# vsxen/inspektor-gadget

Measured on AMD Instinct MI355X. Metric: events aggregated/sec (filter+group-by+top-K) at 1/2/4/8 MI355X; % HBM peak, higher is better.
Workload: dtype u64; 1 GPU; top-tcp: filter family in {AF_INET, AF_INET6}, group-by ip_key_t(saddr,daddr,mntns,pid,comm,lport,dport,family) sum sent/recv, stable top-20 by [-sent,-recv]; events_per_gpu=100000000, keys_per_gpu=1000000, topk=20, groups_per_gpu=991489, batches=21, claims_per_interval=0, parallelism=single GPU

## Files before the change

include/igx.h:

```cpp
#ifndef IGX_H
#define IGX_H

#include <stddef.h>
#include <stdint.h>

#ifdef __cplusplus
extern "C" {
#endif

#define IGX_OK 0
#define IGX_ENOENT (-2)
#define IGX_EIO (-5)
#define IGX_ENOMEM (-12)
#define IGX_EINVAL (-22)
#define IGX_ENOSPC (-28)
#define IGX_ENOTSUP (-95)

enum igx_kind {
    IGX_KIND_INT = 0,
    IGX_KIND_UINT = 1,
    IGX_KIND_FLOAT = 2,
    IGX_KIND_BYTES = 3,
    IGX_KIND_BOOL = 4,
    IGX_KIND_OTHER = 5
// ... 142 lines not shown
int igx_groupby_finalize(igx_table *t, igx_table_view *view);
typedef struct {
    uint32_t form;
    uint32_t region;
    uint32_t part_left;
    uint32_t exact_left;
    uint32_t sm_probers;
    uint32_t loaders;
    uint64_t rows;
    uint32_t miss_permille;
    uint32_t persist;
    uint64_t claims;
    uint64_t gen_keys;
} igx_groupby_info_t;
int igx_groupby_info(igx_table *t, igx_groupby_info_t *out);
int igx_groupby_rowplan(igx_table *t);
int igx_groupby_rowplan_match(const uint32_t *key_widths, uint32_t nkeys, const igx_agg *aggs,
                              uint32_t naggs, const igx_col *cols, uint32_t ncols,
                              const uint32_t *key_cols, const igx_pred *preds, uint32_t npreds,
                              const uint8_t *valid, uint32_t idx_col);
int igx_groupby_finalize_async(igx_table *t, igx_table_view *view);
int igx_groupby_wait(igx_table *t, uint64_t *n_groups);
int igx_groupby_gather(igx_table *t, const uint32_t *idx, uint64_t k, uint8_t *out_rows);
int igx_groupby_select_ge(igx_table *t, uint32_t agg, uint64_t threshold, uint32_t *out_slots,
                          uint64_t cap, uint64_t *d_count);
int igx_groupby_lookup(igx_table *t, const uint8_t *keys, uint32_t key_stride, uint64_t n,
                       uint8_t *out_rows, uint8_t *found);
int igx_groupby_reset(igx_table *t);
enum igx_gb_mode { IGX_GB_AUTO = 0, IGX_GB_CACHED = 1, IGX_GB_DIRECT = 2, IGX_GB_PART = 3 };
int igx_groupby_set_mode(igx_table *t, uint32_t mode);
// ... 188 lines not shown
```

inspektor-gadget_amd/_abi.py:

```python
import ctypes as C
import os

HERE = os.path.dirname(os.path.abspath(__file__))
LIB_PATH = os.environ.get("IGX_LIB") or os.path.join(HERE, "libigx.so")
if os.environ.get("IGX_LIB"):
    import sys as _sys
    print(f"inspektor-gadget_amd: IGX_LIB={LIB_PATH}", file=_sys.stderr, flush=True)

IGX_OK = 0
IGX_ENOENT = -2
IGX_EIO = -5
IGX_ENOMEM = -12
IGX_EINVAL = -22
IGX_ENOSPC = -28
IGX_ENOTSUP = -95

KIND_INT, KIND_UINT, KIND_FLOAT, KIND_BYTES, KIND_BOOL, KIND_OTHER = range(6)
CMP_EQ, CMP_REGEX, CMP_LT, CMP_LE, CMP_GT, CMP_GE, CMP_IN = range(7)
COL_VIRTUAL, COL_EXTRACTOR = 1, 2
NO_COL = 0xFFFFFFFF
MAX_REF = 256
AGG_COUNT, AGG_SUM = 0, 1
FILTER_ANY, FILTER_NIL_MATCH = 1, 2
GB_AUTO, GB_CACHED, GB_DIRECT, GB_PART = 0, 1, 2, 3
# ... 19 lines not shown
    _fields_ = [("col", C.c_uint32), ("cmp", C.c_uint32), ("negate", C.c_uint32),
                ("ref_len", C.c_uint32), ("ref", C.c_uint8 * MAX_REF),
                ("guard_col", C.c_uint32), ("guard_len", C.c_uint32), ("guard_ref", C.c_uint8 * 8)]


class SortKey(C.Structure):
    _fields_ = [("ptr", C.c_void_p), ("width", C.c_uint32), ("kind", C.c_uint32),
                ("desc", C.c_uint32), ("col", C.c_uint32)]


class GroupbyInfo(C.Structure):
    _fields_ = [("form", C.c_uint32), ("region", C.c_uint32), ("part_left", C.c_uint32),
                ("exact_left", C.c_uint32), ("sm_probers", C.c_uint32), ("loaders", C.c_uint32),
                ("rows", C.c_uint64), ("miss_permille", C.c_uint32), ("persist", C.c_uint32),
                ("claims", C.c_uint64), ("gen_keys", C.c_uint64)]


class Agg(C.Structure):
    _fields_ = [("kind", C.c_uint32), ("col", C.c_uint32), ("cond_col", C.c_uint32),
                ("out_width", C.c_uint32), ("cond_val", C.c_uint64), ("divisor", C.c_uint64)]


class TableView(C.Structure):
    _fields_ = [("n_groups", C.c_uint64), ("n_slots", C.c_uint64), ("key_bytes", C.c_uint32),
                ("key_stride", C.c_uint32), ("val_stride", C.c_uint32), ("naggs", C.c_uint32),
                ("keys", C.c_void_p),
                ("aggs", C.c_void_p * 16), ("first_idx", C.c_void_p), ("groups", C.c_void_p),
                ("d_n_groups", C.c_void_p)]


# ... 60 lines not shown
                              C.POINTER(SortKey), C.POINTER(_U32), C.POINTER(_U32)]),
    ("igx_sort_perm", _I, [_VP, C.POINTER(SortKey), _U32, _U64, _VP, _VP, _VP]),
    ("igx_sort_perm_ex", _I, [_VP, C.POINTER(SortKey), _U32, _U64, _VP, _VP, _VP, _VP]),
    ("igx_sort_perm_dn", _I, [_VP, C.POINTER(SortKey), _U32, _U64, _VP, _VP, _VP, _VP, _VP]),
    ("igx_topk", _I, [_VP, C.POINTER(SortKey), _U32, _U64, _VP, _U32, _VP]),
    ("igx_groupby_create", _I, [_VP, C.POINTER(_U32), _U32, C.POINTER(Agg), _U32, _U64,
                                C.POINTER(_VP)]),
    ("igx_groupby_update", _I, [_VP, C.POINTER(Col), _U32, C.POINTER(_U32), C.POINTER(Pred),
                                _U32, _U64, _U64]),
    ("igx_groupby_update_ex", _I, [_VP, C.POINTER(Col), _U32, C.POINTER(_U32), C.POINTER(Pred),
                                   _U32, _VP, _U32, _U64, _U64]),
    ("igx_groupby_finalize", _I, [_VP, C.POINTER(TableView)]),
    ("igx_groupby_finalize_async", _I, [_VP, C.POINTER(TableView)]),
    ("igx_groupby_wait", _I, [_VP, C.POINTER(C.c_uint64)]),
    ("igx_groupby_info", _I, [_VP, C.POINTER(GroupbyInfo)]),
    ("igx_groupby_rowplan", _I, [_VP]),
    ("igx_groupby_rowplan_match", _I, [C.POINTER(_U32), _U32, C.POINTER(Agg), _U32, C.POINTER(Col), _U32,
                                       C.POINTER(_U32), C.POINTER(Pred), _U32, _VP, _U32]),
    ("igx_groupby_gather", _I, [_VP, _VP, _U64, _VP]),
    ("igx_groupby_select_ge", _I, [_VP, _U32, _U64, _VP, _U64, _VP]),
    ("igx_groupby_lookup", _I, [_VP, _VP, _U32, _U64, _VP, _VP]),
    ("igx_groupby_sort", _I, [_VP, C.POINTER(TSortKey), _U32, _U32, _VP]),
    ("igx_segment_fsum", _I, [_VP, _VP, _U32, _U32, _VP, _U64, _VP, _VP, _U32, _VP]),
    ("igx_ip_text", _I, [_VP, _VP, _U32, _VP, _U32, _VP, _U64, _VP]),
    ("igx_groupby_reset", _I, [_VP]),
    ("igx_groupby_set_mode", _I, [_VP, _U32]),
    ("igx_groupby_destroy", _I, [_VP]),
    ("igx_groupby_debug_counts", _I, [_VP, _VP]),
    ("igx_groupby_topk_counts", _I, [_VP, _VP]),
    ("igx_np_mark", _I, [_VP, _VP, _VP, _VP, _VP, _U64, _VP]),
# ... 76 lines not shown
```

inspektor-gadget_amd/csrc/k_gb_cached.hip:

```cpp
#include "k_gb_table.h"

namespace {

constexpr uint32_t ST_EMPTY = 0xFFFFFFFFu;
constexpr uint32_t ST_BUSY = 0xFFFFFFFEu;
constexpr uint32_t GHOST = 1024;

template <int KW>
struct LdsCache {
    static constexpr int KP = (KW + 3) & ~3;
    uint32_t *tag;
    uint32_t *st;
    uint32_t *key;
    uint64_t *agg;
    uint64_t *first;
    uint32_t *ghost;
    uint32_t E;
    uint32_t nsets;
};

template <int KW>
__device__ __forceinline__ bool lds_key_eq(const LdsCache<KW> &c, uint32_t e, const uint32_t (&k)[KW]) {
    constexpr int NQ = LdsCache<KW>::KP / 4;
    const uint4 *p = reinterpret_cast<const uint4 *>(c.key) + (uint64_t)e * (LdsCache<KW>::KP / 4);
// ... 180 lines not shown
        ++lines;
    }
    const uint64_t nlive = (uint64_t)__popcll(__ballot(live));
    if (lane == 0) {
        atomicAdd(a.dbg_cnt + base, (unsigned long long)nlive);
        atomicAdd(a.dbg_cnt + base + 1, (unsigned long long)nmin);
        atomicAdd(a.dbg_cnt + base + 2, (unsigned long long)recs);
        atomicAdd(a.dbg_cnt + base + 3, (unsigned long long)lines);
    }
}

template <bool DBG>
__device__ __forceinline__ void ring_serve(const GbArgs &a, const Ring &r, uint32_t lane) {
    uint32_t head = 0;
    [[maybe_unused]] uint32_t prev_last = 0xFFFFFFFFu;
    for (;;) {
        const uint32_t t = __hip_atomic_load(&r.ctl[0], __ATOMIC_ACQUIRE, __HIP_MEMORY_SCOPE_WORKGROUP);
        if (t == head) {
            if (__hip_atomic_load(&r.ctl[2], __ATOMIC_ACQUIRE, __HIP_MEMORY_SCOPE_WORKGROUP) == NWAVES - 1 - a.nl &&
                __hip_atomic_load(&r.ctl[0], __ATOMIC_ACQUIRE, __HIP_MEMORY_SCOPE_WORKGROUP) == head)
                break;
            __builtin_amdgcn_s_sleep(2);
            if (DBG && (a.dbg & 65536u) && lane == 0) atomicAdd(a.dbg_cnt + 7, 1ull);
            continue;
        }
        const uint32_t n = min(t - head, 64u);
        uint32_t slot = 0xFFFFFFFFu, what = 0;
        if (lane < n) {
            const uint32_t p = head + lane;
            uint64_t w;
            uint32_t spins = 0;
            while (((uint32_t)((w = __hip_atomic_load(reinterpret_cast<uint64_t *>(&r.lo[p % ARING]),
                                                      __ATOMIC_ACQUIRE, __HIP_MEMORY_SCOPE_WORKGROUP)) >> 32) &
                    ~15u) != ring_lap(p)) {
                __builtin_amdgcn_s_sleep(1);
                if (++spins > SPIN_LIMIT) { atomicOr(a.err, 16u); break; }
            }
            const uint64_t val = r.hi[p % ARING];
            slot = (uint32_t)w;
            what = (uint32_t)(w >> 32) & 15u;
            if (DBG && (a.dbg & 131072u)) {
                if (what == WHAT_MIN) *rec_first(a, slot) = val;
                else *rec_agg(a, slot, (int)what) = val;
            } else if (!(DBG && (a.dbg & 4u))) {
                if (what == WHAT_MIN) gmin(rec_first(a, slot), val);
                else gadd(rec_agg(a, slot, (int)what), val);
            }
        }
        if (DBG && (a.dbg & 262144u)) {
            const bool live = lane < n;
            atomics_account(a, live, slot, what == WHAT_MIN, lane, 8);
            for (uint32_t g = 0; g < 3; ++g) {
                const uint32_t sh = 5 - g;
                uint64_t todo = __ballot(live);
                uint64_t cnt = 0;
                while (todo) {
                    const uint32_t l = (uint32_t)__ffsll((long long)todo) - 1;
                    const uint32_t s0 = __shfl(slot, (int)l), k0 = __shfl(what == WHAT_MIN ? 1u : 0u, (int)l);
                    todo &= ~__ballot(live && slot == s0 && (what == WHAT_MIN ? 1u : 0u) == k0 && (lane >> sh) == (l >> sh));
                    ++cnt;
                }
                if (lane == 0) atomicAdd(a.dbg_cnt + 13 + g, (unsigned long long)cnt);
            }
            const uint32_t first_slot = __shfl(slot, 0), last_slot = __shfl(slot, (int)(n - 1));
            if (lane == 0 && first_slot == prev_last) atomicAdd(a.dbg_cnt + 12, 1ull);
            prev_last = last_slot;
        }
        head += n;
        if (lane == 0) __hip_atomic_store(&r.ctl[1], head, __ATOMIC_RELEASE, __HIP_MEMORY_SCOPE_WORKGROUP);
    }
}

constexpr uint32_t MRING = 256;

template <int KW, int NA>
struct MissRing {
    static constexpr int KQ = LdsCache<KW>::KP / 4;
    static constexpr int EQ = KQ + 1 + (NA + 1) / 2;
    uint4 *cell;
    uint32_t *seq;
    uint32_t *ctl;
    uint32_t *err;
    unsigned long long *waits;
};
// ... 794 lines not shown
    (void)igx_groupby_reset(st);
    GbArgs b = a;
    b.n = S;
    b.naggs = 1;
    b.vcount[0] = 1;
    b.hascond[0] = 0;
    b.valid = a.valid;
    bind_records(st, b);
    b.dbg = 0;
    b.sm = 0;
    b.direct = 0;
    b.nl = NL_DEFAULT;
    b.seeds = nullptr;
    b.seed_gep = nullptr;
    b.nseeds = 0;
    st->rows_fed = S;
    st->fin_since_update = false;
    st->interval_direct = st->interval_part = false;
    st->occb_dirty = true;
    launch_gb_as<L, false, 2, true>(ctx, b, (uint32_t)std::max<uint64_t>(1, std::min<uint64_t>((S + GTB - 1) / GTB,
                                                                                           (uint64_t)ctx->num_cus)));
    IGX_HIP(ctx, hipGetLastError());
    int rc = igx_groupby_finalize_async(st, nullptr);
    if (rc) return rc;
    igx_tsortkey key{};
    key.src = IGX_TSRC_AGG;
    key.index = 0;
    key.desc = 1;
    rc = igx_groupby_sort(st, &key, 1, E, t->seed_slots);
    if (rc) return rc;
// ... 40 lines not shown
```

inspektor-gadget_amd/csrc/k_gb_table.h:

```cpp
#pragma once

#include <algorithm>
#include <cstdlib>
#include <cstring>
#include <type_traits>
#include <string>
#include <utility>
#include <vector>

#include <thread>

#include "k_common.h"

#ifndef IGX_GB_STREAM_NT
#define IGX_GB_STREAM_NT 1
#endif
#if IGX_GB_STREAM_NT
#define IGX_STREAM_LOAD(p) __builtin_nontemporal_load(p)
#else
#define IGX_STREAM_LOAD(p) (*(p))
#endif
template <bool NT, class T>
__device__ __forceinline__ T stream_ld(const T *p) {
    if constexpr (NT) return IGX_STREAM_LOAD(p);
// ... 65 lines not shown
    uint32_t vrec_words;
    uint32_t vrec_total;
    uint32_t *err;
    uint32_t *occ;
    uint8_t *occb;
    uint64_t ep;
    uint64_t *gen;
    uint64_t rmask;
    uint32_t sshift;
    uint32_t max_probe;
    uint32_t dbg;
    unsigned long long *dbg_cnt;
    const uint32_t *seeds;
    const uint64_t *seed_gep;
    uint32_t nseeds;
};

__device__ __forceinline__ uint32_t nh_const(int i) {
    return 0x9E3779B9u * (uint32_t)(2 * i + 1) + 0x7F4A7C15u;
}

template <int KW>
__device__ __forceinline__ uint64_t hash_key(const uint32_t (&k)[KW]) {
    uint64_t h = 0x243F6A8885A308D3ull ^ (uint64_t)KW;
#pragma unroll
    for (int w = 0; w < KW; w += 2) {
        const uint32_t a = k[w] + nh_const(w);
        const uint32_t b = ((w + 1 < KW) ? k[w + 1] : 0u) + nh_const(w + 1);
        h += (uint64_t)a * (uint64_t)b;
    }
    h ^= h >> 33;
// ... 606 lines not shown
    uint32_t miss_pm = 0;
    bool rowplan_on = true;
    int rowplan_last = 0;
    uint32_t mode = IGX_GB_AUTO;
    uint32_t direct_left = 0;
    uint32_t region_off = 0;
    bool interval_region = false;
    bool interval_direct = false;
    bool interval_part = false;
    uint32_t *p_recs = nullptr;
    size_t p_recs_bytes = 0;
    uint32_t *p_cnt = nullptr;
    size_t p_cnt_bytes = 0;
    uint8_t *p_mask = nullptr;
    size_t p_mask_bytes = 0;
    uint64_t host_groups = 0;
    uint64_t *fin_host = nullptr;
    uint64_t *fin_dev = nullptr;
    uint64_t fin_seq = 0;
    bool fin_pending = false;
    int fin_status = 0;
    uint64_t fin_status_seq = 0;
    struct {
        uint64_t rows_fed;
        bool direct, part, region, probe;
        uint64_t sampled;
    } fin_snap{};
    bool interval_probe = false;
    uint64_t probe_rows = 0;
    unsigned long long *dbg_cnt = nullptr;
// ... 77 lines not shown

inline int grow(igx_ctx *ctx, void **p, size_t *have, size_t need) {
    if (*have >= need) return IGX_OK;
    IGX_HIP(ctx, hipStreamSynchronize(ctx->stream));
    (void)hipFree(*p);
    *p = nullptr;
    *have = 0;
    IGX_HIP(ctx, hipMalloc(p, need));
    *have = need;
    return IGX_OK;
}

int gb_launch_cached(igx_table *t, GbArgs &a, uint32_t blocks);
int gb_launch_estimate(igx_table *t, const GbArgs &a, uint32_t blocks, uint64_t nsample);
int gb_seeds_compute(igx_table *t, const GbArgs &a);
int gb_launch_direct(igx_table *t, GbArgs &a);
int gb_launch_part(igx_table *t, GbArgs &a);
void gb_cached_load();
void gb_direct_load();
void gb_part_load();
int fin_collect(igx_table *t, uint64_t *n_groups);
```

inspektor-gadget_amd/csrc/k_groupby.hip:

```cpp
#include "k_gb_table.h"

namespace {

__global__ void k_table_clear(uint8_t *krec, uint32_t krec_len, uint32_t koff, uint64_t ns) {
    const uint64_t stride = (uint64_t)gridDim.x * blockDim.x;
    for (uint64_t i = (uint64_t)blockIdx.x * blockDim.x + threadIdx.x; i < ns; i += stride)
        *reinterpret_cast<uint4 *>(krec + i * krec_len + koff) = make_uint4(0, 0, 0, 0);
}

constexpr int CT = 256 * 32;

__global__ __launch_bounds__(256) void k_occ_from_tags(const uint8_t *__restrict__ krec, uint32_t krec_len,
                                                       uint32_t koff, uint64_t ns, uint64_t ep,
                                                       uint32_t *__restrict__ occ) {
    const uint64_t w = (uint64_t)blockIdx.x * 256 + threadIdx.x;
    if (w * 32 >= ns) return;
    uint32_t m = 0;
#pragma unroll 8
    for (uint32_t b = 0; b < 32; ++b) {
        const uint64_t s = w * 32 + b;
        const uint64_t t = s < ns ? *reinterpret_cast<const uint64_t *>(krec + s * krec_len + koff) : 0;
        m |= ((t & EP_MAX) == ep ? 1u : 0u) << b;
    }
    occ[w] |= m;
// ... 30 lines not shown

__device__ __forceinline__ void fin_export(const uint32_t *err, uint64_t total, uint64_t *host, uint64_t seq, uint64_t ep) {
    const uint64_t e0 = *reinterpret_cast<const volatile uint64_t *>(err);
    const uint64_t e1 = *reinterpret_cast<const volatile uint64_t *>(err + 2);
    volatile uint64_t *gen = reinterpret_cast<volatile uint64_t *>(const_cast<uint32_t *>(err)) + GEN_WORD;
    const bool fresh = gen[0] == ep;
    const uint64_t claims = fresh ? total : gen[2];
    const uint64_t keys = (uint32_t)e0 ? ~0ull : (fresh ? total : gen[1] + claims);
    gen[1] = keys;
    gen[2] = 0;
    __hip_atomic_store(host, e0, __ATOMIC_RELAXED, __HIP_MEMORY_SCOPE_SYSTEM);
    __hip_atomic_store(host + 1, e1, __ATOMIC_RELAXED, __HIP_MEMORY_SCOPE_SYSTEM);
    __hip_atomic_store(host + 2, total, __ATOMIC_RELAXED, __HIP_MEMORY_SCOPE_SYSTEM);
    __hip_atomic_store(host + 4, claims, __ATOMIC_RELAXED, __HIP_MEMORY_SCOPE_SYSTEM);
    __hip_atomic_store(host + 5, keys, __ATOMIC_RELAXED, __HIP_MEMORY_SCOPE_SYSTEM);
    __threadfence_system();
    __hip_atomic_store(host + 3, seq, __ATOMIC_RELEASE, __HIP_MEMORY_SCOPE_SYSTEM);
}

__global__ __launch_bounds__(1024) void k_slots_scan(uint32_t *__restrict__ v, uint64_t m, uint64_t *__restrict__ total,
                                                     const uint32_t *__restrict__ err, uint64_t *__restrict__ host,
                                                     uint64_t seq, uint64_t ep) {
    __shared__ uint32_t part[1024];
    const uint64_t per = (m + 1023) / 1024;
    const uint64_t b = threadIdx.x * per, e = min(m, b + per);
    uint32_t s = 0;
    for (uint64_t i = b; i < e; ++i) s += v[i];
    part[threadIdx.x] = s;
    __syncthreads();
    for (int d = 1; d < 1024; d <<= 1) {
// ... 67 lines not shown
    const uint32_t *groups;
    const uint64_t *ng;
    uint64_t *vrec;
    uint32_t vw, may;
};
__global__ __launch_bounds__(256) void k_reset_clear(uint32_t *__restrict__ occ, uint64_t nwords,
                                                     uint32_t *__restrict__ err, uint4 *__restrict__ occb,
                                                     uint64_t nb16, ResetGen rg) {
    const uint64_t i = (uint64_t)blockIdx.x * 256 + threadIdx.x;
    const uint64_t stride = (uint64_t)gridDim.x * 256;
    const uint64_t n4 = nwords / 4;
    for (uint64_t q = i; q < n4; q += stride) reinterpret_cast<uint4 *>(occ)[q] = make_uint4(0, 0, 0, 0);
    for (uint64_t q = i; q < nb16; q += stride) occb[q] = make_uint4(0, 0, 0, 0);
    if (i < (nwords & 3)) occ[n4 * 4 + i] = 0;
    if (i < 4) err[i] = 0;
    const bool cont = rg.may && rg.gen[1] <= rg.limit;
    if (cont) {
        constexpr int RU = 8;
        const uint64_t ng = *rg.ng;
        const uint32_t qs = rg.vw == 1 ? 0u : (uint32_t)__builtin_ctz(rg.vw / 2);
        const uint64_t total = ng << qs;
        const uint32_t *__restrict__ groups = rg.groups;
        uint64_t *__restrict__ vrec = rg.vrec;
        for (uint64_t j0 = i; j0 < total; j0 += RU * stride) {
            uint32_t slot[RU];
#pragma unroll
            for (int u = 0; u < RU; ++u) {
                const uint64_t j = j0 + u * stride;
                slot[u] = j < total ? groups[j >> qs] : 0u;
            }
// ... 175 lines not shown
    t->cap = capacity;
    uint64_t slotf = 8;
    if (const char *d = std::getenv("IGX_GB_SLOTF")) slotf = std::max<uint64_t>(5, std::strtoul(d, nullptr, 0));
    uint64_t ns = 1024;
    while (ns * 4 < slotf * capacity) ns <<= 1;
    t->nslots = ns;
    t->sbits = (uint32_t)__builtin_ctzll(ns);
    t->rbits = std::max<uint32_t>(10, t->sbits > 14 ? t->sbits - 14 : 0);
    t->wide = ns * t->krec_len >= (1ull << 32);
    if (const char *d = std::getenv("IGX_GB_WIDE"))
        t->wide = t->wide || std::strtoul(d, nullptr, 0) != 0;
    const uint64_t tiles = (ns + CT - 1) / CT;
    hipError_t e = hipMalloc(&t->krec, ns * t->krec_len);
    if (e == hipSuccess) e = hipMemsetAsync(t->krec, 0, ns * t->krec_len, ctx->stream);
    if (e == hipSuccess) e = hipMalloc(&t->vrec, ns * t->vrec_len);
    if (e == hipSuccess) e = hipMalloc(&t->err, 64);
    if (e == hipSuccess) e = hipMemsetAsync(t->err, 0, 64, ctx->stream);
    if (e == hipSuccess) e = hipMalloc(&t->groups, ns * 4);
    if (e == hipSuccess) e = hipMalloc(&t->tile_cnt, tiles * 4);
    t->occ_words = (ns + 31) / 32;
    if (e == hipSuccess) e = hipMalloc(&t->occ, t->occ_words * 4);
    if (e == hipSuccess) e = hipMalloc(&t->occb, t->occ_words * 32);
    if (e == hipSuccess) e = hipMemsetAsync(t->occb, 0, t->occ_words * 32, ctx->stream);
    if (e == hipSuccess) t->n_groups = reinterpret_cast<uint64_t *>(t->err + 4);
    if (e == hipSuccess) e = hipMalloc(&t->dbg_cnt, 256);
    if (e == hipSuccess)
        e = hipHostMalloc(reinterpret_cast<void **>(&t->fin_host), 64, hipHostMallocMapped | hipHostMallocCoherent);
    if (e == hipSuccess) e = hipHostGetDevicePointer(reinterpret_cast<void **>(&t->fin_dev), t->fin_host, 0);
    if (e == hipSuccess) std::fill(t->fin_host, t->fin_host + 8, 0ull);
    if (e == hipSuccess) e = hipMemsetAsync(t->dbg_cnt, 0, 256, ctx->stream);
    if (e != hipSuccess) {
        igx_groupby_destroy(t);
        return igx_fail(ctx, IGX_ENOMEM, "groupby_create: %s", hipGetErrorString(e));
    }
    if (const char *m = std::getenv("IGX_GB_MODE")) {
        const unsigned long v = std::strtoul(m, nullptr, 0);
        if (v <= IGX_GB_PART && !(t->wide && v == IGX_GB_CACHED)) t->mode = (uint32_t)v;
    }
    if (const char *m = std::getenv("IGX_GB_PERSIST")) t->persist = std::strtoul(m, nullptr, 0) != 0;
    if (const char *m = std::getenv("IGX_GB_SEED")) t->seed_on = std::strtoul(m, nullptr, 0) != 0;
    *out = t;
    return igx_groupby_reset(t);
}

// ... 48 lines not shown
    (void)hipFree(t->krec);
    (void)hipFree(t->vrec);
    (void)hipFree(t->err);
    (void)hipFree(t->groups);
    (void)hipFree(t->tile_cnt);
    (void)hipFree(t->occ);
    (void)hipFree(t->occb);
    (void)hipFree(t->dbg_cnt);
    (void)hipFree(t->seeds);
    (void)hipFree(t->seed_slots);
    (void)hipFree(t->seed_gep);
    if (t->seed_tab) igx_groupby_destroy(t->seed_tab);
    (void)hipFree(t->p_recs);
    (void)hipFree(t->p_cnt);
    (void)hipFree(t->p_mask);
    for (auto &h : t->tk) (void)hipFree(h.slots);
    (void)hipFree(t->tk_state);
    for (auto *p : t->text) (void)hipFree(p);
    if (t->fin_host) (void)hipHostFree(t->fin_host);
    delete t;
    return IGX_OK;
}

constexpr uint64_t DIRECT_MISS_PCT = 90;
constexpr uint64_t MORE_PROBERS_ON_PM = 390;
constexpr uint64_t MORE_PROBERS_OFF_PM = 370;
constexpr uint32_t DIRECT_RUN = 16;
constexpr uint64_t PROBE_ROWS = 16u << 20;
constexpr uint32_t SEED_EVERY = 16;
constexpr uint64_t SEED_MIN_ROWS = 8u << 20;
// ... 37 lines not shown
                uint32_t every = SEED_EVERY;
                if (const char *e = std::getenv("IGX_GB_SEED_EVERY"))
                    every = std::max<uint32_t>(1, (uint32_t)std::strtoul(e, nullptr, 0));
                if (gb_seeds_compute(t, a) == IGX_OK) t->seed_left = every;
                else t->nseeds = 0;
            }
            --t->seed_left;
            t->interval_seeded = t->nseeds > 0;
        }
    }
    if (t->interval_seeded) {
        a.seeds = t->seeds;
        a.seed_gep = t->seed_gep;
        a.nseeds = t->nseeds;
    }
    return gb_launch_cached(t, a, blocks);
}

extern "C" int igx_groupby_set_mode(igx_table *t, uint32_t mode) {
    if (!t) return IGX_EINVAL;
    if (mode > IGX_GB_PART) return igx_fail(t->ctx, IGX_EINVAL, "groupby_set_mode: mode %u", mode);
    if (t->wide && mode == IGX_GB_CACHED)
        return igx_fail(t->ctx, IGX_ENOTSUP, "groupby_set_mode: the cached form is not available on a wide table "
                                             "(%llu slots x %u B of key records; 64-bit record addressing)",
                        (unsigned long long)t->nslots, t->krec_len);
    t->mode = mode;
    t->direct_left = 0;
    return IGX_OK;
}

extern "C" int igx_groupby_update(igx_table *t, const igx_col *cols, uint32_t ncols, const uint32_t *key_cols,
// ... 363 lines not shown
    for (uint32_t x = 0; x < 16; ++x) view->aggs[x] = x < t->naggs ? t->vrec + 1 + x : nullptr;
    view->first_idx = t->vrec;
    view->groups = t->groups;
    view->d_n_groups = t->n_groups;
}

static int fin_apply(igx_table *t) {
    igx_ctx *ctx = t->ctx;
    const uint64_t *h = t->fin_host;
    const uint32_t err = reinterpret_cast<const uint32_t *>(h)[0];
    const uint64_t misses = h[1];
    const uint64_t ng = h[2];
    const uint32_t spilled = reinterpret_cast<const uint32_t *>(h)[1];
    t->claims_last = h[4];
    t->gen_keys = h[5];
    if (h[4] == ng || h[5] == ~0ull) t->seed_left = 0;
    const auto &f = t->fin_snap;
    if (spilled && f.region) t->region_off = DIRECT_RUN + 1;
    t->host_groups = ng;
    if (f.rows_fed >= 1000000 && !f.direct && !f.part) {
        t->prefer_sm = misses * 10 > f.rows_fed * 7;
        t->miss_pm = (uint32_t)(misses * 1000 / f.rows_fed);
        t->more_probers = t->miss_pm > (t->more_probers ? MORE_PROBERS_OFF_PM : MORE_PROBERS_ON_PM);
        if (t->mode == IGX_GB_AUTO && misses * 100 > f.rows_fed * DIRECT_MISS_PCT) t->direct_left = DIRECT_RUN;
    }
    if (f.probe && f.sampled && t->mode == IGX_GB_AUTO && misses * 100 > f.sampled * DIRECT_MISS_PCT)
        t->direct_left = DIRECT_RUN;
    if (err) return igx_fail(ctx, IGX_ENOSPC, "groupby: table full or probe failure (err=%u)", err);
    if (ng > t->cap)
        return igx_fail(ctx, IGX_ENOSPC, "groupby: %llu distinct keys exceed capacity %llu",
// ... 67 lines not shown
extern "C" int igx_groupby_info(igx_table *t, igx_groupby_info_t *out) {
    if (!t || !out) return IGX_EINVAL;
    std::memset(out, 0, sizeof *out);
    if (t->rows_fed)
        out->form = t->interval_part ? IGX_GB_PART : (t->interval_direct ? IGX_GB_DIRECT : IGX_GB_CACHED);
    out->region = t->interval_part && t->interval_region ? 1u : 0u;
    out->part_left = t->direct_left;
    out->exact_left = t->region_off;
    out->sm_probers = t->prefer_sm ? 1u : 0u;
    out->loaders = t->more_probers ? NL_DEFAULT - 1 : NL_DEFAULT;
    out->miss_permille = t->miss_pm;
    out->rows = t->rows_fed;
    out->claims = t->claims_last;
    out->gen_keys = t->gen_keys;
    out->persist = t->persist ? 1u : 0u;
    return IGX_OK;
}

static uint64_t agg_out_mask(const igx_table *t, uint32_t x) {
    const uint32_t ow = t->aggs[x].out_width;
    return (ow == 0 || ow >= 8) ? ~0ull : ((1ull << (8 * ow)) - 1);
}
static AggMasks agg_masks(const igx_table *t) {
    AggMasks am{};
    for (uint32_t x = 0; x < t->naggs; ++x) {
        const uint64_t m = agg_out_mask(t, x);
        am.m[2 * x] = (uint32_t)m;
        am.m[2 * x + 1] = (uint32_t)(m >> 32);
    }
    return am;
// ... 197 lines not shown
```

inspektor-gadget_amd/engine.py:

```python
import ctypes as C
import os
import math

from . import _abi
from ._abi import Agg, Col, Pred, SortKey, TableView, IgxError
from .runtime import context, ptr, col_of, dtype_kind, torch_mod

TCP_FIELDS = (("saddr", "u8x16"), ("daddr", "u8x16"), ("mntns", "u64"), ("pid", "u32"),
              ("comm", "u8x16"), ("lport", "u16"), ("dport", "u16"), ("family", "u16"),
              ("size", "u32"), ("dir", "u8"))
OPEN_FIELDS = (("pid", "u32"), ("uid", "u32"), ("mntns", "u64"), ("comm", "u8x16"),
               ("ret", "i64"), ("fd", "i64"), ("err", "i64"), ("path", "u32"))
BIO_FIELDS = (("dev", "u32"), ("cont", "u32"), ("delta", "i64"))
NP_FIELDS = (("src", "u32"), ("peer", "u32"), ("port", "u16"), ("pkt", "u8"), ("type", "u8"),
             ("proto", "u8"), ("hostip", "u32"), ("raddr", "u32"))
FILE_FIELDS = (("inode", "u64"), ("dev", "u32"), ("pid", "u32"), ("tid", "u32"), ("op", "u8"),
               ("count", "u32"))


def zipf_cdf(G: int, s: float):
    import numpy as np
    k = np.arange(1, G + 1, dtype=np.float64)
    c = np.cumsum(k ** (-s))
    c /= c[-1]
# ... 171 lines not shown
                                              ptr(valid), _abi.NO_COL if idx_col is None else idx_col,
                                              n, base_idx))

    def wait(self):
        n = C.c_uint64()
        self.ctx.check(self.ctx.L.igx_groupby_wait(self.h, C.byref(n)))
        if getattr(self, "fin", None) is not None:
            self.fin["n_groups"] = n.value
        return n.value

    def info(self):
        from ._abi import GroupbyInfo
        v = GroupbyInfo()
        self.ctx.check(self.ctx.L.igx_groupby_info(self.h, C.byref(v)))
        return {f: getattr(v, f) for f, _ in GroupbyInfo._fields_ if f != "pad"}

    def rowplan(self):
        return int(self.ctx.L.igx_groupby_rowplan(self.h))

    def reset(self):
        self.ctx.check(self.ctx.L.igx_groupby_reset(self.h))

    def set_mode(self, mode):
        self.ctx.check(self.ctx.L.igx_groupby_set_mode(self.h, mode))

    def finalize(self, sync=True):
        v = TableView()
        if sync:
            self.ctx.check(self.ctx.L.igx_groupby_finalize(self.h, C.byref(v)))
        else:
# ... 576 lines not shown
```

Before: 34.49 billion events/s.

## Log ring-server aggregate adds and reduce them via bucketed partition pass

Rather than issuing a scattered global atomic add per aggregate update in the cached ring server, the server writes compact (slot, agg, value) records to a per-workgroup log. Two follow-up kernels partition the log by slot bucket in shared memory and then reduce each bucket with LDS atomics before one global add per touched accumulator. Records that are too large or that overflow the log or a bucket fall back to direct atomics, and the fallback counts are reported through a new stats API. This aims to replace random HBM atomic traffic with streaming writes and reads, at the cost of extra buffers, two extra kernel launches and more total bytes moved.

```diff
diff --git a/include/igx.h b/include/igx.h
--- a/include/igx.h
+++ b/include/igx.h
@@ -180,6 +180,13 @@
     uint64_t gen_keys;
 } igx_groupby_info_t;
 int igx_groupby_info(igx_table *t, igx_groupby_info_t *out);
+typedef struct {
+    uint64_t logged;
+    uint64_t fallback_value;
+    uint64_t fallback_log_full;
+    uint64_t fallback_bucket_full;
+} igx_groupby_log_stats_t;
+int igx_groupby_log_stats(igx_table *t, igx_groupby_log_stats_t *out);
 int igx_groupby_rowplan(igx_table *t);
 int igx_groupby_rowplan_match(const uint32_t *key_widths, uint32_t nkeys, const igx_agg *aggs,
                               uint32_t naggs, const igx_col *cols, uint32_t ncols,
diff --git a/inspektor-gadget_amd/_abi.py b/inspektor-gadget_amd/_abi.py
--- a/inspektor-gadget_amd/_abi.py
+++ b/inspektor-gadget_amd/_abi.py
@@ -57,6 +57,11 @@
                 ("exact_left", C.c_uint32), ("sm_probers", C.c_uint32), ("loaders", C.c_uint32),
                 ("rows", C.c_uint64), ("miss_permille", C.c_uint32), ("persist", C.c_uint32),
                 ("claims", C.c_uint64), ("gen_keys", C.c_uint64)]
+
+
+class GroupbyLogStats(C.Structure):
+    _fields_ = [("logged", C.c_uint64), ("fallback_value", C.c_uint64),
+                ("fallback_log_full", C.c_uint64), ("fallback_bucket_full", C.c_uint64)]
 
 
 class Agg(C.Structure):
@@ -147,6 +152,7 @@
     ("igx_groupby_finalize_async", _I, [_VP, C.POINTER(TableView)]),
     ("igx_groupby_wait", _I, [_VP, C.POINTER(C.c_uint64)]),
     ("igx_groupby_info", _I, [_VP, C.POINTER(GroupbyInfo)]),
+    ("igx_groupby_log_stats", _I, [_VP, C.POINTER(GroupbyLogStats)]),
     ("igx_groupby_rowplan", _I, [_VP]),
     ("igx_groupby_rowplan_match", _I, [C.POINTER(_U32), _U32, C.POINTER(Agg), _U32, C.POINTER(Col), _U32,
                                        C.POINTER(_U32), C.POINTER(Pred), _U32, _VP, _U32]),
diff --git a/inspektor-gadget_amd/csrc/k_gb_cached.hip b/inspektor-gadget_amd/csrc/k_gb_cached.hip
--- a/inspektor-gadget_amd/csrc/k_gb_cached.hip
+++ b/inspektor-gadget_amd/csrc/k_gb_cached.hip
@@ -218,6 +218,9 @@
 __device__ __forceinline__ void ring_serve(const GbArgs &a, const Ring &r, uint32_t lane) {
     uint32_t head = 0;
     [[maybe_unused]] uint32_t prev_last = 0xFFFFFFFFu;
+    const bool logging = !DBG && a.log != nullptr;
+    uint64_t *lg = a.log + (uint64_t)blockIdx.x * a.log_cap;
+    uint32_t lpos = 0, n_logged = 0, n_value = 0, n_full = 0;
     for (;;) {
         const uint32_t t = __hip_atomic_load(&r.ctl[0], __ATOMIC_ACQUIRE, __HIP_MEMORY_SCOPE_WORKGROUP);
         if (t == head) {
@@ -229,6 +232,7 @@
             continue;
         }
         const uint32_t n = min(t - head, 64u);
+        const bool room = logging && lpos + n <= a.log_cap;
         uint32_t slot = 0xFFFFFFFFu, what = 0;
         if (lane < n) {
             const uint32_t p = head + lane;
@@ -243,12 +247,28 @@
             const uint64_t val = r.hi[p % ARING];
             slot = (uint32_t)w;
             what = (uint32_t)(w >> 32) & 15u;
-            if (DBG && (a.dbg & 131072u)) {
+            bool logged = false;
+            if (logging && what != WHAT_MIN) {
+                const bool small = (val >> 32) == 0;
+                const bool fits = small && slot < LOG_SLOT_LIMIT;
+                if (!small) ++n_value;
+                if (fits && !room) ++n_full;
+                logged = fits && room;
+                n_logged += logged ? 1u : 0u;
+            }
+            if (room)
+                __builtin_nontemporal_store(logged ? log_record(slot, what, (uint32_t)val) : ~0ull, lg + lpos + lane);
+            if (logged) {
+            } else if (DBG && (a.dbg & 131072u)) {
                 if (what == WHAT_MIN) *rec_first(a, slot) = val;
                 else *rec_agg(a, slot, (int)what) = val;
             } else if (!(DBG && (a.dbg & 4u))) {
                 if (what == WHAT_MIN) gmin(rec_first(a, slot), val);
+#ifndef IGX_DIAG_NO_SERVER_ADDS
                 else gadd(rec_agg(a, slot, (int)what), val);
+#else
+                else asm volatile("" ::"v"(val));
+#endif
             }
         }
         if (DBG && (a.dbg & 262144u)) {
@@ -271,7 +291,22 @@
             prev_last = last_slot;
         }
         head += n;
+        if (room) lpos += n;
         if (lane == 0) __hip_atomic_store(&r.ctl[1], head, __ATOMIC_RELEASE, __HIP_MEMORY_SCOPE_WORKGROUP);
+    }
+    if (logging) {
+        for (int o = 32; o > 0; o >>= 1) {
+            n_logged += __shfl_xor(n_logged, o);
+            n_value += __shfl_xor(n_value, o);
+            n_full += __shfl_xor(n_full, o);
+        }
+        if (lane == 0) {
+            a.log_cnt[blockIdx.x] = lpos;
+            unsigned long long *st = reinterpret_cast<unsigned long long *>(a.err) + LOG_STAT_WORD;
+            if (n_logged) atomicAdd(st, (unsigned long long)n_logged);
+            if (n_value) atomicAdd(st + 1, (unsigned long long)n_value);
+            if (n_full) atomicAdd(st + 2, (unsigned long long)n_full);
+        }
     }
 }
 
@@ -1096,6 +1131,7 @@
     b.seeds = nullptr;
     b.seed_gep = nullptr;
     b.nseeds = 0;
+    b.log = nullptr;
     st->rows_fed = S;
     st->fin_since_update = false;
     st->interval_direct = st->interval_part = false;
diff --git a/inspektor-gadget_amd/csrc/k_gb_log.hip b/inspektor-gadget_amd/csrc/k_gb_log.hip
--- /dev/null
+++ b/inspektor-gadget_amd/csrc/k_gb_log.hip
@@ -0,0 +1,228 @@
+#include "k_gb_table.h"
+
+namespace {
+
+constexpr uint32_t LOG_TILE = 16384;
+constexpr uint32_t LOG_TB = 1024;
+constexpr uint32_t LOG_RPT = LOG_TILE / LOG_TB;
+constexpr uint32_t LOG_NB_MAX = 1024;
+constexpr size_t LOG_ACC_BYTES = 128 * 1024;
+constexpr uint32_t LOG_CNT_WORDS = 4096;
+constexpr uint32_t LOG_BCNT_OFF = LOG_CNT_WORDS - LOG_NB_MAX;
+constexpr uint64_t LOG_COLD_ROWS = 8192;
+constexpr uint64_t LOG_BUCKET_SLACK = 16384;
+
+struct LogArgs {
+    const uint64_t *log;
+    const uint32_t *wcnt;
+    uint64_t *bk;
+    uint32_t *bcnt;
+    uint64_t *vrec;
+    uint32_t *err;
+    uint32_t cap, nwg, bcap, nb;
+    uint32_t bshift;
+    uint32_t spb;
+    uint32_t naggs, vrec_words;
+    uint64_t nslots;
+};
+
+__device__ __forceinline__ unsigned long long *log_agg(const LogArgs &a, uint32_t slot, uint32_t x) {
+    return reinterpret_cast<unsigned long long *>(a.vrec + (uint64_t)slot * a.vrec_words + 1 + x);
+}
+
+__global__ __launch_bounds__(LOG_TB) void k_gbl_part(LogArgs a) {
+    extern __shared__ uint64_t sorted[];
+    __shared__ uint32_t cnt[LOG_NB_MAX], off[LOG_NB_MAX], gbase[LOG_NB_MAX], wsum[LOG_TB / 64];
+    const uint32_t tid = threadIdx.x, lane = tid & 63, wave = tid >> 6;
+    const uint32_t wg = blockIdx.x % a.nwg, ti = blockIdx.x / a.nwg;
+    const uint32_t have = min(a.wcnt[wg], a.cap);
+    const uint64_t start = (uint64_t)ti * LOG_TILE;
+    if (start >= have) return;
+    const uint32_t m = (uint32_t)min((uint64_t)LOG_TILE, have - start);
+    const uint64_t *src = a.log + (uint64_t)wg * a.cap + start;
+    cnt[tid] = 0;
+    __syncthreads();
+    uint64_t rec[LOG_RPT];
+    uint32_t rank[LOG_RPT];
+#pragma unroll
+    for (uint32_t k = 0; k < LOG_RPT; ++k) {
+        const uint32_t i = k * LOG_TB + tid;
+        rec[k] = i < m ? __builtin_nontemporal_load(src + i) : ~0ull;
+    }
+#pragma unroll
+    for (uint32_t k = 0; k < LOG_RPT; ++k) {
+        const uint32_t hi = (uint32_t)(rec[k] >> 32);
+        rank[k] = 0;
+        if (hi == LOG_NULL_HI) continue;
+        if ((hi >> 2) >= a.nslots || (hi & 3u) >= a.naggs) {
+            atomicOr(a.err, 16u);
+            rec[k] = ~0ull;
+            continue;
+        }
+        rank[k] = atomicAdd(&cnt[(hi >> 2) >> a.bshift], 1u);
+    }
+    __syncthreads();
+    const uint32_t c = cnt[tid];
+    gbase[tid] = c ? atomicAdd(&a.bcnt[tid], c) : 0u;
+    uint32_t inc = c;
+#pragma unroll
+    for (int d = 1; d < 64; d <<= 1) {
+        const uint32_t u = __shfl_up(inc, d);
+        if ((int)lane >= d) inc += u;
+    }
+    if (lane == 63) wsum[wave] = inc;
+    __syncthreads();
+    uint32_t before = 0;
+    for (uint32_t w = 0; w < wave; ++w) before += wsum[w];
+    off[tid] = before + inc - c;
+    __syncthreads();
+#pragma unroll
+    for (uint32_t k = 0; k < LOG_RPT; ++k) {
+        const uint32_t hi = (uint32_t)(rec[k] >> 32);
+        if (hi != LOG_NULL_HI) sorted[off[(hi >> 2) >> a.bshift] + rank[k]] = rec[k];
+    }
+    __syncthreads();
+    const uint32_t total = off[LOG_NB_MAX - 1] + cnt[LOG_NB_MAX - 1];
+    uint32_t nfull = 0;
+    for (uint32_t i = tid; i < total; i += LOG_TB) {
+        const uint64_t r = sorted[i];
+        const uint32_t hi = (uint32_t)(r >> 32), b = (hi >> 2) >> a.bshift;
+        const uint64_t j = (uint64_t)gbase[b] + (i - off[b]);
+        if (j < a.bcap) {
+            __builtin_nontemporal_store(r, a.bk + (uint64_t)b * a.bcap + j);
+        } else {
+            gadd(log_agg(a, hi >> 2, hi & 3u), (unsigned long long)(uint32_t)r);
+            ++nfull;
+        }
+    }
+    if (__ballot(nfull != 0)) {
+        for (int o = 32; o > 0; o >>= 1) nfull += __shfl_xor(nfull, o);
+        if (lane == 0)
+            atomicAdd(reinterpret_cast<unsigned long long *>(a.err) + LOG_STAT_WORD + 3, (unsigned long long)nfull);
+    }
+}
+
+__global__ __launch_bounds__(LOG_TB) void k_gbl_reduce(LogArgs a) {
+    extern __shared__ uint64_t acc[];
+    const uint32_t tid = threadIdx.x, b = blockIdx.x;
+    const uint32_t nacc = a.spb * a.naggs;
+    const uint32_t have = min(a.bcnt[b], a.bcap);
+    if (!have) return;
+    for (uint32_t q = tid; q < nacc; q += LOG_TB) acc[q] = 0;
+    __syncthreads();
+    const uint64_t *src = a.bk + (uint64_t)b * a.bcap;
+    constexpr uint32_t U = 4;
+    for (uint32_t i0 = tid; i0 < have; i0 += U * LOG_TB) {
+        uint64_t r[U];
+#pragma unroll
+        for (uint32_t u = 0; u < U; ++u) {
+            const uint32_t i = i0 + u * LOG_TB;
+            r[u] = i < have ? __builtin_nontemporal_load(src + i) : ~0ull;
+        }
+#pragma unroll
+        for (uint32_t u = 0; u < U; ++u) {
+            const uint32_t hi = (uint32_t)(r[u] >> 32);
+            if (hi == LOG_NULL_HI) continue;
+            const uint32_t q = ((hi >> 2) & (a.spb - 1)) * a.naggs + (hi & 3u);
+            atomicAdd(reinterpret_cast<unsigned long long *>(&acc[q]), (unsigned long long)(uint32_t)r[u]);
+        }
+    }
+    __syncthreads();
+    for (uint32_t q = tid; q < nacc; q += LOG_TB) {
+        const uint64_t v = acc[q];
+        const uint32_t s = q / a.naggs, x = q - s * a.naggs;
+        if (v) gadd(log_agg(a, b * a.spb + s, x), (unsigned long long)v);
+    }
+    if (tid == 0) a.bcnt[b] = 0;
+}
+
+uint32_t log_spb(const igx_table *t) {
+    uint32_t spb = 1;
+    while ((size_t)spb * 2 * t->naggs * 8 <= LOG_ACC_BYTES) spb <<= 1;
+    return (uint32_t)std::min<uint64_t>(spb, t->nslots);
+}
+
+}
+
+int gb_log_prepare(igx_table *t, GbArgs &a, uint32_t blocks) {
+    a.log = nullptr;
+    a.log_cnt = nullptr;
+    a.log_cap = 0;
+    if (t->wide || t->naggs < 1 || t->naggs > 4 || a.direct || a.dbg) return IGX_OK;
+    if (t->nslots & (t->nslots - 1)) return IGX_OK;
+    if (const char *d = std::getenv("IGX_GB_LOG"))
+        if (std::strtoul(d, nullptr, 0) == 0) return IGX_OK;
+    const uint32_t spb = log_spb(t);
+    const uint64_t nb = t->nslots / spb;
+    if (nb > LOG_NB_MAX || blocks > LOG_BCNT_OFF || t->nslots > LOG_SLOT_LIMIT) return IGX_OK;
+    const uint64_t rows_wg = (a.n + blocks - 1) / blocks;
+    uint64_t cap = (rows_wg / 2 + std::min<uint64_t>(rows_wg, LOG_COLD_ROWS) * t->naggs + 63) & ~63ull;
+    cap = std::max<uint64_t>(cap, 64);
+    if (const char *d = std::getenv("IGX_GB_LOG_CAP")) cap = std::max<uint64_t>(1, std::strtoull(d, nullptr, 0));
+    uint64_t bcap = (uint64_t)blocks * cap / nb * 5 / 4 + LOG_BUCKET_SLACK;
+    if (const char *d = std::getenv("IGX_GB_LOG_BCAP")) bcap = std::max<uint64_t>(1, std::strtoull(d, nullptr, 0));
+    if (cap >= (1ull << 31) || bcap >= (1ull << 31)) return IGX_OK;
+    igx_ctx *ctx = t->ctx;
+    if (!t->lg_cnt) {
+        if (hipMalloc(&t->lg_cnt, LOG_CNT_WORDS * 4) != hipSuccess) {
+            (void)hipGetLastError();
+            t->lg_cnt = nullptr;
+            return IGX_OK;
+        }
+        IGX_HIP(ctx, hipMemsetAsync(t->lg_cnt, 0, LOG_CNT_WORDS * 4, ctx->stream));
+    }
+    size_t have = t->lg_recs_bytes;
+    if (grow(ctx, reinterpret_cast<void **>(&t->lg_recs), &have, (size_t)blocks * cap * 8) != IGX_OK) {
+        (void)hipGetLastError();
+        t->lg_recs_bytes = 0;
+        return IGX_OK;
+    }
+    t->lg_recs_bytes = have;
+    have = t->lg_bk_bytes;
+    if (grow(ctx, reinterpret_cast<void **>(&t->lg_bk), &have, (size_t)nb * bcap * 8) != IGX_OK) {
+        (void)hipGetLastError();
+        t->lg_bk_bytes = 0;
+        return IGX_OK;
+    }
+    t->lg_bk_bytes = have;
+    a.log = t->lg_recs;
+    a.log_cnt = t->lg_cnt;
+    a.log_cap = (uint32_t)cap;
+    return IGX_OK;
+}
+
+int gb_log_launch(igx_table *t, const GbArgs &a, uint32_t blocks) {
+    if (!a.log) return IGX_OK;
+    igx_ctx *ctx = t->ctx;
+    static bool attr = false;
+    if (!attr) {
+        (void)hipFuncSetAttribute(reinterpret_cast<const void *>(k_gbl_part), hipFuncAttributeMaxDynamicSharedMemorySize,
+                                  LOG_TILE * 8);
+        (void)hipFuncSetAttribute(reinterpret_cast<const void *>(k_gbl_reduce),
+                                  hipFuncAttributeMaxDynamicSharedMemorySize, LOG_ACC_BYTES);
+        attr = true;
+    }
+    LogArgs l{};
+    l.log = a.log;
+    l.wcnt = a.log_cnt;
+    l.bk = t->lg_bk;
+    l.bcnt = t->lg_cnt + LOG_BCNT_OFF;
+    l.vrec = t->vrec;
+    l.err = t->err;
+    l.cap = a.log_cap;
+    l.nwg = blocks;
+    l.spb = log_spb(t);
+    l.nb = (uint32_t)(t->nslots / l.spb);
+    l.bshift = (uint32_t)__builtin_ctz(l.spb);
+    l.naggs = t->naggs;
+    l.vrec_words = t->vrec_len / 8;
+    l.nslots = t->nslots;
+    l.bcap = (uint32_t)std::min<uint64_t>(t->lg_bk_bytes / 8 / l.nb, (1u << 31) - 1);
+    if (const char *d = std::getenv("IGX_GB_LOG_BCAP"))
+        l.bcap = (uint32_t)std::min<uint64_t>(l.bcap, std::max<uint64_t>(1, std::strtoull(d, nullptr, 0)));
+    const uint32_t tiles = (a.log_cap + LOG_TILE - 1) / LOG_TILE;
+    hipLaunchKernelGGL(k_gbl_part, dim3(blocks * tiles), dim3(LOG_TB), LOG_TILE * 8, ctx->stream, l);
+    hipLaunchKernelGGL(k_gbl_reduce, dim3(l.nb), dim3(LOG_TB), (size_t)l.spb * l.naggs * 8, ctx->stream, l);
+    IGX_HIP(ctx, hipGetLastError());
+    return IGX_OK;
+}
diff --git a/inspektor-gadget_amd/csrc/k_gb_table.h b/inspektor-gadget_amd/csrc/k_gb_table.h
--- a/inspektor-gadget_amd/csrc/k_gb_table.h
+++ b/inspektor-gadget_amd/csrc/k_gb_table.h
@@ -103,7 +103,17 @@
     const uint32_t *seeds;
     const uint64_t *seed_gep;
     uint32_t nseeds;
-};
+    uint32_t log_cap;
+    uint64_t *log;
+    uint32_t *log_cnt;
+};
+
+constexpr uint32_t LOG_NULL_HI = 0xFFFFFFFFu;
+constexpr uint32_t LOG_SLOT_LIMIT = (1u << 30) - 1;
+constexpr int LOG_STAT_WORD = 8;
+__device__ __forceinline__ uint64_t log_record(uint32_t slot, uint32_t agg, uint32_t value) {
+    return ((uint64_t)((slot << 2) | agg) << 32) | value;
+}
 
 __device__ __forceinline__ uint32_t nh_const(int i) {
     return 0x9E3779B9u * (uint32_t)(2 * i + 1) + 0x7F4A7C15u;
@@ -740,6 +750,12 @@
     size_t p_cnt_bytes = 0;
     uint8_t *p_mask = nullptr;
     size_t p_mask_bytes = 0;
+    uint64_t *lg_recs = nullptr;
+    size_t lg_recs_bytes = 0;
+    uint64_t *lg_bk = nullptr;
+    size_t lg_bk_bytes = 0;
+    uint32_t *lg_cnt = nullptr;
+    uint64_t log_last[4] = {};
     uint64_t host_groups = 0;
     uint64_t *fin_host = nullptr;
     uint64_t *fin_dev = nullptr;
@@ -847,6 +863,8 @@
 int gb_launch_cached(igx_table *t, GbArgs &a, uint32_t blocks);
 int gb_launch_estimate(igx_table *t, const GbArgs &a, uint32_t blocks, uint64_t nsample);
 int gb_seeds_compute(igx_table *t, const GbArgs &a);
+int gb_log_prepare(igx_table *t, GbArgs &a, uint32_t blocks);
+int gb_log_launch(igx_table *t, const GbArgs &a, uint32_t blocks);
 int gb_launch_direct(igx_table *t, GbArgs &a);
 int gb_launch_part(igx_table *t, GbArgs &a);
 void gb_cached_load();
diff --git a/inspektor-gadget_amd/csrc/k_groupby.hip b/inspektor-gadget_amd/csrc/k_groupby.hip
--- a/inspektor-gadget_amd/csrc/k_groupby.hip
+++ b/inspektor-gadget_amd/csrc/k_groupby.hip
@@ -68,6 +68,10 @@
     __hip_atomic_store(host + 2, total, __ATOMIC_RELAXED, __HIP_MEMORY_SCOPE_SYSTEM);
     __hip_atomic_store(host + 4, claims, __ATOMIC_RELAXED, __HIP_MEMORY_SCOPE_SYSTEM);
     __hip_atomic_store(host + 5, keys, __ATOMIC_RELAXED, __HIP_MEMORY_SCOPE_SYSTEM);
+    for (int x = 0; x < 4; ++x)
+        __hip_atomic_store(host + LOG_STAT_WORD + x,
+                           *(reinterpret_cast<const volatile uint64_t *>(err) + LOG_STAT_WORD + x), __ATOMIC_RELAXED,
+                           __HIP_MEMORY_SCOPE_SYSTEM);
     __threadfence_system();
     __hip_atomic_store(host + 3, seq, __ATOMIC_RELEASE, __HIP_MEMORY_SCOPE_SYSTEM);
 }
@@ -165,6 +169,7 @@
     for (uint64_t q = i; q < nb16; q += stride) occb[q] = make_uint4(0, 0, 0, 0);
     if (i < (nwords & 3)) occ[n4 * 4 + i] = 0;
     if (i < 4) err[i] = 0;
+    if (i >= 2 * LOG_STAT_WORD && i < 2 * LOG_STAT_WORD + 8) err[i] = 0;
     const bool cont = rg.may && rg.gen[1] <= rg.limit;
     if (cont) {
         constexpr int RU = 8;
@@ -370,8 +375,8 @@
     hipError_t e = hipMalloc(&t->krec, ns * t->krec_len);
     if (e == hipSuccess) e = hipMemsetAsync(t->krec, 0, ns * t->krec_len, ctx->stream);
     if (e == hipSuccess) e = hipMalloc(&t->vrec, ns * t->vrec_len);
-    if (e == hipSuccess) e = hipMalloc(&t->err, 64);
-    if (e == hipSuccess) e = hipMemsetAsync(t->err, 0, 64, ctx->stream);
+    if (e == hipSuccess) e = hipMalloc(&t->err, 128);
+    if (e == hipSuccess) e = hipMemsetAsync(t->err, 0, 128, ctx->stream);
     if (e == hipSuccess) e = hipMalloc(&t->groups, ns * 4);
     if (e == hipSuccess) e = hipMalloc(&t->tile_cnt, tiles * 4);
     t->occ_words = (ns + 31) / 32;
@@ -381,9 +386,9 @@
     if (e == hipSuccess) t->n_groups = reinterpret_cast<uint64_t *>(t->err + 4);
     if (e == hipSuccess) e = hipMalloc(&t->dbg_cnt, 256);
     if (e == hipSuccess)
-        e = hipHostMalloc(reinterpret_cast<void **>(&t->fin_host), 64, hipHostMallocMapped | hipHostMallocCoherent);
+        e = hipHostMalloc(reinterpret_cast<void **>(&t->fin_host), 128, hipHostMallocMapped | hipHostMallocCoherent);
     if (e == hipSuccess) e = hipHostGetDevicePointer(reinterpret_cast<void **>(&t->fin_dev), t->fin_host, 0);
-    if (e == hipSuccess) std::fill(t->fin_host, t->fin_host + 8, 0ull);
+    if (e == hipSuccess) std::fill(t->fin_host, t->fin_host + 16, 0ull);
     if (e == hipSuccess) e = hipMemsetAsync(t->dbg_cnt, 0, 256, ctx->stream);
     if (e != hipSuccess) {
         igx_groupby_destroy(t);
@@ -462,6 +467,9 @@
     (void)hipFree(t->p_recs);
     (void)hipFree(t->p_cnt);
     (void)hipFree(t->p_mask);
+    (void)hipFree(t->lg_recs);
+    (void)hipFree(t->lg_bk);
+    (void)hipFree(t->lg_cnt);
     for (auto &h : t->tk) (void)hipFree(h.slots);
     (void)hipFree(t->tk_state);
     for (auto *p : t->text) (void)hipFree(p);
@@ -529,7 +537,10 @@
         a.seed_gep = t->seed_gep;
         a.nseeds = t->nseeds;
     }
-    return gb_launch_cached(t, a, blocks);
+    int rc = gb_log_prepare(t, a, blocks);
+    if (rc) return rc;
+    if ((rc = gb_launch_cached(t, a, blocks))) return rc;
+    return gb_log_launch(t, a, blocks);
 }
 
 extern "C" int igx_groupby_set_mode(igx_table *t, uint32_t mode) {
@@ -923,6 +934,7 @@
     const uint32_t spilled = reinterpret_cast<const uint32_t *>(h)[1];
     t->claims_last = h[4];
     t->gen_keys = h[5];
+    for (int x = 0; x < 4; ++x) t->log_last[x] = h[LOG_STAT_WORD + x];
     if (h[4] == ng || h[5] == ~0ull) t->seed_left = 0;
     const auto &f = t->fin_snap;
     if (spilled && f.region) t->region_off = DIRECT_RUN + 1;
@@ -1020,6 +1032,15 @@
     out->claims = t->claims_last;
     out->gen_keys = t->gen_keys;
     out->persist = t->persist ? 1u : 0u;
+    return IGX_OK;
+}
+
+extern "C" int igx_groupby_log_stats(igx_table *t, igx_groupby_log_stats_t *out) {
+    if (!t || !out) return IGX_EINVAL;
+    out->logged = t->log_last[0];
+    out->fallback_value = t->log_last[1];
+    out->fallback_log_full = t->log_last[2];
+    out->fallback_bucket_full = t->log_last[3];
     return IGX_OK;
 }
 
diff --git a/inspektor-gadget_amd/engine.py b/inspektor-gadget_amd/engine.py
--- a/inspektor-gadget_amd/engine.py
+++ b/inspektor-gadget_amd/engine.py
@@ -209,6 +209,12 @@
         v = GroupbyInfo()
         self.ctx.check(self.ctx.L.igx_groupby_info(self.h, C.byref(v)))
         return {f: getattr(v, f) for f, _ in GroupbyInfo._fields_ if f != "pad"}
+
+    def log_stats(self):
+        from ._abi import GroupbyLogStats
+        v = GroupbyLogStats()
+        self.ctx.check(self.ctx.L.igx_groupby_log_stats(self.h, C.byref(v)))
+        return {f: getattr(v, f) for f, _ in GroupbyLogStats._fields_}
 
     def rowplan(self):
         return int(self.ctx.L.igx_groupby_rowplan(self.h))
```

Measured after the change: 35.71 billion events/s (median of 6 runs). 1.04x the previous value.
